# scrose/pylc

Measured on AMD Instinct MI355X. Metric: 512x512 tiles/sec fwd+bwd (DeepLabV3+/ResNet101, 9-class), higher is better.
Workload: dtype f32; 1 GPU; DeepLabV3+ ResNet101 OS16, 3-ch 512x512 tiles, 9 classes, CE+Dice+Focal, clip 0.5 + AdamW, bs=32/GPU (BASELINE.json configs[2]); global_batch=32, parallelism=dp1, conv_arithmetic=f16x3 split (fp32-grade), rccl_ranks=0, wgrad_queue=compute stream, sync_bn=True, activation_format=fp16 planes between BatchNorm and conv kernels (4 B/element)

## Files before the change

### include/pylc_hip.h

```cpp
#ifndef PYLC_HIP_H
#define PYLC_HIP_H

#include <stddef.h>
#include <stdint.h>

#ifdef __cplusplus
extern "C" {
#endif

#define PYLC_OK 0
#define PYLC_ERR_ARG 1
#define PYLC_ERR_HIP 2
#define PYLC_ERR_WORKSPACE 3
#define PYLC_ERR_UNSUPPORTED 4

const char* pylc_last_error(void);
int pylc_abi_version(void);
int pylc_experimental_build(void);
int pylc_init(void);

typedef struct PylcConvDesc {
    int B, H, W;
    int Cin, Cout;
    int R, S;
// ... 280 lines not shown
                            float* losses, void* stream);
int pylc_multiloss_bwd(const float* logits, int pitch, const int64_t* target, long long N, int C,
                       const float* class_weights, const float* stats, double n_global,
                       float w_ce, float w_dice, float w_focal, const float* grad_scale,
                       float* dlogits, int dpitch, unsigned int* amax_bits, void* stream);

size_t pylc_sqnorm_workspace_floats(long long n);
int pylc_grad_norm_clip(const float* g, long long n, float max_norm, float* out2, float* workspace, void* stream);
int pylc_adamw_step(float* p, const float* g, float* m, float* v, long long n, const float* coef,
                    float lr, float beta1, float beta2, float eps, float weight_decay, int step, void* stream);
int pylc_adamw_step_ranges(float* p, const float* g, float* m, float* v, long long n, const float* coef,
                           float lr, float beta1, float beta2, float eps, float weight_decay, int step,
                           const long long* seg_offsets, int seg_count, unsigned int* seg_amax_bits, void* stream);
int pylc_sgd_step(float* p, const float* g, float* buf, long long n, const float* coef, float lr, float momentum,
                  int step, void* stream);

int pylc_dropout(const float* x, int x_pitch, float* out, int out_pitch, long long M, int C, float p,
                 uint64_t seed, void* stream);

#ifdef PYLC_EXPERIMENTAL
int pylc_stream_create_cu_mask(int n_cus, int from_top, void** stream_out);
int pylc_stream_destroy(void* stream);
#endif

int pylc_debug_set_big_tile(int mode);
int pylc_debug_pp_flags(int flags);
int pylc_debug_stagger(int units);
int pylc_debug_dw_tiles(int on);
int pylc_debug_wgrad_m16(int on);
int pylc_debug_wgrad_dma(int on);
int pylc_debug_wgrad_acc1(int on);
int pylc_debug_wgrad_sets(int mode);
int pylc_debug_wgrad_flags(int flags);
int pylc_debug_wgrad_max_steps(int steps);
int pylc_debug_pp_stamps(unsigned long long* buf);

#define PYLC_COMM_ID_BYTES 128
int pylc_comm_available(void);
int pylc_comm_unique_id(void* id_out);
int pylc_comm_init(const void* id, int rank, int world, void** comm_out);
int pylc_comm_allreduce(void* comm, void* buf, long long count, int dtype, void* stream);
int pylc_comm_syncbn_reduce(void* comm, double* moments, int channels, void* stream);
int pylc_comm_destroy(void* comm);

#ifdef __cplusplus
}
#endif
#endif
```

### pylc_amd/csrc/conv_common.h

```cpp
#pragma once
#include "common.h"
#include <type_traits>

namespace pylc {

typedef float f32x4 __attribute__((ext_vector_type(4)));
typedef float f32x16 __attribute__((ext_vector_type(16)));

typedef __bf16 bf16x8 __attribute__((ext_vector_type(8)));

typedef _Float16 f16x8 __attribute__((ext_vector_type(8)));
typedef _Float16 f16x2 __attribute__((ext_vector_type(2)));
typedef float f32x2 __attribute__((ext_vector_type(2)));

constexpr int LDB = 80;

__device__ __forceinline__ void split3(const float (&x)[4], uint2& p0, uint2& p1, uint2& p2) {
    unsigned u0[4], u1[4], u2[4];
#pragma unroll
    for (int e = 0; e < 4; ++e) {
        u0[e] = __float_as_uint(x[e]);
        const float r1 = x[e] - __uint_as_float(u0[e] & 0xFFFF0000u);
        u1[e] = __float_as_uint(r1);
        const float r2 = r1 - __uint_as_float(u1[e] & 0xFFFF0000u);
// ... 106 lines not shown
__device__ __forceinline__ float row_sum16(float v) {
#define PYLC_DPP_ADD(ctrl) v += __builtin_bit_cast(float, __builtin_amdgcn_update_dpp(0, __builtin_bit_cast(int, v), ctrl, 0xF, 0xF, true))
    PYLC_DPP_ADD(0xB1);
    PYLC_DPP_ADD(0x4E);
    PYLC_DPP_ADD(0x141);
    PYLC_DPP_ADD(0x140);
#undef PYLC_DPP_ADD
    return v;
}


struct WgradArgs {
    const float* x;
    const float* dy;
    float* out;
    int M, P, Q;
    int IH, IW, Cin, x_pitch, in_sh, in_sw;
    int TR, TS, dh0, dh_step, dw0, dw_step;
    int N, N_ld, dy_pitch;
    int out_row_stride;
    int tiles_n, tiles_c;
    int splits, m_per_split;
    long long slab_stride;
    const unsigned* amax_dy;
    const unsigned* amax_x;
    long long x_bytes, dy_bytes;
    const void* x_planes;
    const void* dy_planes;
    long long x_plane_stride, dy_plane_stride;
    int nterms;
    int dbg_flags;
};

typedef short s16x4 __attribute__((ext_vector_type(4)));
typedef short s16x8 __attribute__((ext_vector_type(8)));
typedef s16x4 __attribute__((address_space(3))) * lds_s16x4_ptr;

__host__ __device__ constexpr int wg_rowb(int w) { return w * 2 + (w == 32 ? 0 : 64); }

__device__ __forceinline__ bf16x8 tr_frag(const char* p, int rowb) {
    const s16x4 lo = __builtin_amdgcn_ds_read_tr16_b64_v4i16((lds_s16x4_ptr)(p));
    const s16x4 hi = __builtin_amdgcn_ds_read_tr16_b64_v4i16((lds_s16x4_ptr)(p + 4 * rowb));
    const s16x8 v = __builtin_shufflevector(lo, hi, 0, 1, 2, 3, 4, 5, 6, 7);
    return __builtin_bit_cast(bf16x8, v);
}


int launch_wg_pl(WgradArgs& a, int cfg, long long grid, hipStream_t st);
int wgrad_pl_init();

bool takes_pl(const GatherGemmArgs& a);
int launch_gg_pl(GatherGemmArgs& a, hipStream_t st);
int conv_pl_init();
bool takes_stem(const GatherGemmArgs& a);
int launch_stem_fwd(GatherGemmArgs& a, hipStream_t st);
int conv_stem_init();

extern int g_conv_precision;
extern int g_wg_flags;
extern int g_pp_flags;

}
```

### pylc_amd/csrc/conv_igemm.hip

```cpp
#include "conv_common.h"

namespace pylc {

template <int BM, int BN, int WM, int WN, bool CIN4, int PREC>
__global__ __launch_bounds__((BM / WM) * (BN / WN) * 64, 2) void gather_gemm_kernel(const GatherGemmArgs a) {
    constexpr int WAVES_N = BN / WN;
    constexpr int MT = WM / 32, NT = WN / 32;
    constexpr int NTHR = (BM / WM) * (BN / WN) * 64;
    constexpr int RPI = NTHR / 8;
    constexpr int A_IT = BM / RPI, B_IT = BN / RPI;
    static_assert(NTHR == 256 || NTHR == 512, "4 or 8 waves per block");
    static_assert(BM % RPI == 0 && BN % RPI == 0, "tile rows must divide evenly over the loader");
    extern __shared__ __attribute__((aligned(16))) float smem[];
    float* sA = smem;
    float* sB = smem + 2 * BM * LDT;

    const int tile = xcd_remap(blockIdx.x, gridDim.x);
    const int m0 = (tile / a.tiles_n) * BM;
    const int n0 = (tile % a.tiles_n) * BN;
    const int tid = threadIdx.x, lane = tid & 63, wave = tid >> 6;
    const int wave_m = wave / WAVES_N, wave_n = wave % WAVES_N;
    const int v = tid & 7, r0 = tid >> 3;

    int rowh[A_IT], roww[A_IT], rowpix[A_IT];
// ... 1857 lines not shown
        const PylcSlabSum e = tab[lo];
        const long long i = (t - tile_prefix[lo]) * 32 + col;
        f32x4 s = {0.f, 0.f, 0.f, 0.f};
        if (i < e.n4)
            for (int k = sl; k < e.splits; k += 4 * 8) {
                f32x4 v[4];
#pragma unroll
                for (int u = 0; u < 4; ++u) v[u] = *reinterpret_cast<const f32x4*>(e.slabs + (size_t)(k + 8 * u < e.splits ? k + 8 * u : k) * e.slab_stride + 4 * i);
#pragma unroll
                for (int u = 0; u < 4; ++u) { if (k + 8 * u < e.splits) s += v[u]; }
            }
        red[sl][col] = s;
        __syncthreads();
        if (sl == 0 && i < e.n4) {
#pragma unroll
            for (int j = 1; j < 8; ++j) s += red[j][col];
            *reinterpret_cast<f32x4*>(e.dw + 4 * i) = s;
        }
        __syncthreads();
    }
}

extern "C" int pylc_splitk_reduce_batch(const PylcSlabSum* table_dev, const long long* tile_prefix_dev, int n, long long total_tiles, void* stream) {
    PYLC_REQUIRE(table_dev && tile_prefix_dev && n > 0 && total_tiles > 0, "splitk_reduce_batch: bad arguments");
    const int blocks = (int)(total_tiles < 4096 ? total_tiles : 4096);
    hipLaunchKernelGGL(splitk_reduce_batch_kernel, dim3(blocks), dim3(256), 0, as_stream(stream), table_dev, tile_prefix_dev, n, total_tiles);
    PYLC_LAUNCH_CHECK();
    return PYLC_OK;
}

static int wgrad_impl(const PylcConvDesc* d, const float* x, const float* dy, float* dw, float* dbias,
                      void* workspace, size_t workspace_bytes, PylcSlabSum* pending, void* stream);

extern "C" int pylc_conv2d_wgrad(const PylcConvDesc* d, const float* x, const float* dy, float* dw, float* dbias,
                                 void* workspace, size_t workspace_bytes, void* stream) {
    return wgrad_impl(d, x, dy, dw, dbias, workspace, workspace_bytes, nullptr, stream);
}

extern "C" int pylc_conv2d_wgrad_slabs(const PylcConvDesc* d, const float* x, const float* dy, float* dw, void* workspace, size_t workspace_bytes,
                                       PylcSlabSum* pending, void* stream) {
    PYLC_REQUIRE(pending != nullptr, "conv2d_wgrad_slabs: null `pending`");
    return wgrad_impl(d, x, dy, dw, nullptr, workspace, workspace_bytes, pending, stream);
}

static int wgrad_impl(const PylcConvDesc* d, const float* x, const float* dy, float* dw, float* dbias,
                      void* workspace, size_t workspace_bytes, PylcSlabSum* pending, void* stream) {
    if (int rc = check_desc(d)) return rc;
    PYLC_REQUIRE(x && dy && dw, "null pointer");
    PYLC_REQUIRE(dbias == nullptr, "dbias: use pylc_bn_stats on dy (column sums)");
    PYLC_REQUIRE(d->x_fmt == d->dy_fmt, "conv2d_wgrad: x and dy must be in the same format (both fp32 or both fp16 planes; pylc_to_planes converts)");
    hipStream_t st = as_stream(stream);
    const WgradPlan p = plan_wgrad(d);
    const size_t need = p.splits > 1 ? (size_t)p.splits * p.slab * sizeof(float) : 0;
    if (need > workspace_bytes || (need && !workspace))
        return fail(PYLC_ERR_WORKSPACE, "wgrad workspace too small: need %zu bytes, got %zu", need, workspace_bytes);
    PYLC_REQUIRE(p.slab % 4 == 0, "dw size must be a multiple of 4");
    const int T = d->R * d->S;
    WgradArgs a{};
    a.x = x; a.dy = dy; a.out = p.splits > 1 ? static_cast<float*>(workspace) : dw;
    a.P = d->OH; a.Q = d->OW; a.M = d->B * d->OH * d->OW;
    a.IH = d->H; a.IW = d->W; a.Cin = d->Cin; a.x_pitch = d->x_pitch; a.in_sh = a.in_sw = d->stride;
    a.TR = d->R; a.TS = d->S; a.dh0 = -d->pad; a.dh_step = d->dil; a.dw0 = -d->pad; a.dw_step = d->dil;
    a.N = d->Cout; a.N_ld = roundup4(d->Cout); a.dy_pitch = d->y_pitch;
    PYLC_REQUIRE(a.N_ld <= d->y_pitch, "dy pitch must cover roundup4(Cout)");
    a.out_row_stride = T * d->Cin;
    a.tiles_n = p.tiles_n; a.tiles_c = p.tiles_c; a.splits = p.splits; a.m_per_split = p.m_per_split;
    a.slab_stride = p.slab;
    PYLC_REQUIRE(g_conv_precision < 2 || (d->dy_amax && d->x_amax), "f16x3 / fp16 mode: conv2d_wgrad needs dy_amax and x_amax in the descriptor");
    a.x_bytes = (((long long)d->B * d->H * d->W - 1) * d->x_pitch + d->Cin) * 4;
    a.dy_bytes = (((long long)d->B * d->OH * d->OW - 1) * d->y_pitch + a.N_ld) * 4;
    a.amax_dy = d->dy_amax; a.amax_x = d->x_amax;
    const long long grid = (long long)p.tiles_n * p.tiles_c * (p.cin4 ? 1 : T) * p.splits;
    int rc;
    if (d->x_fmt == 1) {
        PYLC_REQUIRE(g_conv_precision >= 2 && !p.cin4 && d->Cout % 8 == 0, "conv2d_wgrad: fp16-plane operands need precision mode 2 or 3, "
                     "a dense geometry and Cout %% 8 == 0");
        a.x_planes = x; a.dy_planes = dy; a.x = nullptr; a.dy = nullptr;
        a.x_plane_stride = planes_stride_rule((long long)d->B * d->H * d->W, d->Cin, d->x_pitch, (g_conv_precision == 3 ? 1 : 2));
        a.dy_plane_stride = planes_stride_rule((long long)d->B * d->OH * d->OW, d->Cout, d->y_pitch, (g_conv_precision == 3 ? 1 : 2));
        a.N_ld = d->Cout;
        a.x_bytes /= 2; a.dy_bytes = (((long long)d->B * d->OH * d->OW - 1) * d->y_pitch + a.N_ld) * 2;
        a.nterms = g_conv_precision == 3 ? 1 : 3;
        rc = launch_wg_pl(a, p.cfg, grid, st);
    } else
    switch (p.cfg) {
        case 0: rc = launch_wg<128, 128, 64, 64, false>(a, grid, st); break;
        case 1: rc = launch_wg<64, 64, 32, 32, false>(a, grid, st); break;
        case 2: rc = launch_wg<32, 128, 32, 32, false>(a, grid, st); break;
        default: rc = launch_wg<64, 64, 32, 32, true>(a, grid, st); break;
    }
    if (rc) return rc;
    if (pending != nullptr) {
        *pending = PylcSlabSum{p.splits > 1 ? static_cast<const float*>(workspace) : nullptr, dw, p.slab / 4, p.slab, p.splits > 1 ? p.splits : 0, 0};
        return PYLC_OK;
    }
    if (p.splits > 1) {
        const long long n4 = p.slab / 4;
        const int blocks = (int)(cdiv<long long>(n4, 32) < 4096 ? cdiv<long long>(n4, 32) : 4096);
        hipLaunchKernelGGL(splitk_reduce_kernel, dim3(blocks), dim3(256), 0, st, static_cast<const float*>(workspace), dw, n4,
                           p.splits, p.slab);
// ... 14 lines not shown
```

### pylc_amd/csrc/wgrad_pl.hip

```cpp
#include "conv_common.h"

namespace pylc {

typedef __attribute__((address_space(3))) void* wg_lds_vptr;
template <int BN, int BC, int WN, int WC, int NTERMS, int FAST, bool ACC1 = false, int SETS = 1, bool M16 = false, bool DMA = false>
__global__ __launch_bounds__(256, ACC1 ? 4 : 2) void wgrad_pl_kernel(const WgradArgs a) {
    static_assert(!DMA || (M16 && SETS == 1), "DMA: the 16x16x32 image only");
    constexpr int NPL = NTERMS == 3 ? 2 : 1;
    constexpr int WAVES_C = BC / WC;
    constexpr int NT = WN / 32, CT = WC / 32;
    static_assert(!M16 || (BN == 128 && BC == 128 && WN == 64 && WC == 64 && !ACC1), "M16: 128 x 128 block tiles, 64 x 64 wave tiles, two accumulator sets");
    constexpr int VA = BN / 8, RA = 256 / VA, IA = 32 / RA > 0 ? 32 / RA : 1;
    constexpr int VB = BC / 8, RB = 256 / VB, IB = 32 / RB > 0 ? 32 / RB : 1;
    constexpr bool A_ALL = RA <= 32, B_ALL = RB <= 32;
    constexpr int ROWA = M16 ? 256 : wg_rowb(BN), ROWB = M16 ? 256 : wg_rowb(BC);
    constexpr int PLA = 32 * ROWA, PLB = 32 * ROWB;
    static_assert((BN / WN) * (BC / WC) == 4, "4 waves per block");
    static_assert(FAST == 1 || FAST == 2, "buffer-load geometry paths only");
    extern __shared__ __attribute__((aligned(16))) float smem[];
    char* sA = reinterpret_cast<char*>(smem);
    char* sB = sA + NPL * PLA;
    constexpr int STG = NPL * (PLA + PLB);

    const int T = a.TR * a.TS;
    int id = (a.dbg_flags & 1) ? (int)blockIdx.x : xcd_remap(blockIdx.x, gridDim.x);
    int tc, tn, tap, split;
    if (a.dbg_flags & 2) {
        split = id % a.splits; id /= a.splits;
        tc = id % a.tiles_c; id /= a.tiles_c;
        tn = id % a.tiles_n; id /= a.tiles_n;
        tap = id;
    } else if (a.dbg_flags & 4) {
        tc = id % a.tiles_c; id /= a.tiles_c;
        tn = id % a.tiles_n; id /= a.tiles_n;
        tap = id % T; id /= T;
        split = id;
    } else if (a.Cin > a.N && !(a.dbg_flags & 8)) {
        tap = id % T; id /= T;
        tn = id % a.tiles_n; id /= a.tiles_n;
        tc = id % a.tiles_c; id /= a.tiles_c;
        split = id;
    } else {
        tap = id % T; id /= T;
        tc = id % a.tiles_c; id /= a.tiles_c;
        tn = id % a.tiles_n; id /= a.tiles_n;
        split = id;
    }
    const int n0 = tn * BN, c0 = tc * BC;
    const int m_begin = split * a.m_per_split;
    const int m_end = min(a.M, m_begin + a.m_per_split);
    const int S = (m_end - m_begin + 31) / 32;

    const int tid = threadIdx.x, lane = tid & 63, wave = tid >> 6;
    const int wave_n = wave / WAVES_C, wave_c = wave % WAVES_C;
    const int va = tid % VA, pra = tid / VA;
    const int vb = tid % VB, prb = tid / VB;
    const int sw_row = ((pra & 3) << 2) | ((pra >> 2) & 3);
    const int va_g = DMA ? (va ^ sw_row) : va, vb_g = DMA ? (vb ^ sw_row) : vb;
    const int dh = a.dh0 + (tap / a.TS) * a.dh_step, dw = a.dw0 + (tap % a.TS) * a.dw_step;
    const bool b_col_ok = c0 + 8 * vb_g < a.Cin && (B_ALL || prb < 32);
    const bool a_col_ok = n0 + 8 * va_g < a.N_ld && (A_ALL || pra < 32);

    f32x16 acc[M16 ? 1 : NT][M16 ? 1 : CT];
    constexpr bool TWO_ACC = NTERMS == 3 && !ACC1;
    f32x16 acc_lo[TWO_ACC && !M16 ? NT : 1][TWO_ACC && !M16 ? CT : 1];
    f32x4 acc16[M16 ? 4 : 1][M16 ? 4 : 1], acc16_lo[M16 && TWO_ACC ? 4 : 1][M16 && TWO_ACC ? 4 : 1];
    if constexpr (M16) {
#pragma unroll
        for (int i = 0; i < 4; ++i)
#pragma unroll
            for (int j = 0; j < 4; ++j) {
                acc16[i][j] = f32x4{0.f, 0.f, 0.f, 0.f};
                if constexpr (TWO_ACC) acc16_lo[i][j] = f32x4{0.f, 0.f, 0.f, 0.f};
            }
    } else {
#pragma unroll
    for (int i = 0; i < NT; ++i)
#pragma unroll
        for (int j = 0; j < CT; ++j)
#pragma unroll
            for (int r = 0; r < 16; ++r) {
                acc[i][j][r] = 0.f;
                if constexpr (TWO_ACC) acc_lo[i][j][r] = 0.f;
            }
    }
    const float scale_a = pow2_scale_for(*a.amax_dy), scale_b = pow2_scale_for(*a.amax_x);

    constexpr unsigned OOB = 0xFFFFFFF0u;
    const bool il_dy = NPL == 2 && planes_il(a.dy_plane_stride), il_x = NPL == 2 && planes_il(a.x_plane_stride);
    const unsigned mdy = (unsigned)__builtin_amdgcn_readfirstlane(il_dy ? 2 : 1), mx = (unsigned)__builtin_amdgcn_readfirstlane(il_x ? 2 : 1);
    auto colh = [](unsigned c, bool il) { return il ? ((c >> 5) << 6) + (c & 31u) : c; };
    const __amdgpu_buffer_rsrc_t rdy0 = __builtin_amdgcn_make_buffer_rsrc(const_cast<void*>(a.dy_planes), 0, (int)((unsigned)a.dy_bytes * mdy), 0x00020000);
    const __amdgpu_buffer_rsrc_t rdy1 = __builtin_amdgcn_make_buffer_rsrc(
        const_cast<char*>(static_cast<const char*>(a.dy_planes) + a.dy_plane_stride * 2), 0, (int)((unsigned)a.dy_bytes * mdy - (il_dy ? 64u : 0u)), 0x00020000);
    const __amdgpu_buffer_rsrc_t rx0 = __builtin_amdgcn_make_buffer_rsrc(const_cast<void*>(a.x_planes), 0, (int)((unsigned)a.x_bytes * mx), 0x00020000);
    const __amdgpu_buffer_rsrc_t rx1 = __builtin_amdgcn_make_buffer_rsrc(
        const_cast<char*>(static_cast<const char*>(a.x_planes) + a.x_plane_stride * 2), 0, (int)((unsigned)a.x_bytes * mx - (il_x ? 64u : 0u)), 0x00020000);

    constexpr int NSET = SETS;
    uint4 ra[NSET][IA][NPL], rb[NSET][IB][NPL];
    int f_mb = m_begin, f_q0 = 0, f_p = 0, f_b = 0;
    unsigned f_va[IA], f_tx[IB];
    int f_wc[IB];
    int g_q[FAST == 2 ? IB : 1], g_p[FAST == 2 ? IB : 1], g_b[FAST == 2 ? IB : 1];
    if constexpr (FAST == 2) {
#pragma unroll
        for (int i = 0; i < IB; ++i) {
            const int m = m_begin + prb + RB * i;
            g_q[i] = m % a.Q;
            const int t = m / a.Q;
            g_p[i] = t % a.P;
            g_b[i] = t / a.P;
        }
    }
    {
        f_q0 = m_begin % a.Q;
        const int t = m_begin / a.Q;
        f_p = t % a.P;
        f_b = t / a.P;
#pragma unroll
        for (int i = 0; i < IA; ++i) f_va[i] = a_col_ok ? ((unsigned)(pra + RA * i) * (unsigned)a.dy_pitch * mdy + colh((unsigned)(n0 + 8 * va_g), il_dy)) * 2u : OOB;
#pragma unroll
        for (int i = 0; i < IB; ++i) {
            f_tx[i] = ((unsigned)((prb + RB * i) * a.in_sw) * (unsigned)a.x_pitch * mx + colh((unsigned)(c0 + 8 * vb_g), il_x)) * 2u;
            f_wc[i] = (prb + RB * i) * a.in_sw + dw;
        }
    }
    char* dma_a = nullptr; char* dma_b = nullptr;
    if constexpr (DMA) { dma_a = sA + (4 * wave) * 256; dma_b = sB + (4 * wave) * 256; }
    auto ldp = [&](const __amdgpu_buffer_rsrc_t& r0, const __amdgpu_buffer_rsrc_t& r1, unsigned voff, unsigned soff, uint4 (&dst)[NPL], char* lds0, int plb) {
        if constexpr (DMA) {
            __builtin_amdgcn_raw_ptr_buffer_load_lds(r0, (wg_lds_vptr)lds0, 16, voff, soff, 0, 0);
            if constexpr (NPL == 2) __builtin_amdgcn_raw_ptr_buffer_load_lds(r1, (wg_lds_vptr)(lds0 + plb), 16, voff, soff, 0, 0);
        } else {
            dst[0] = __builtin_bit_cast(uint4, __builtin_amdgcn_raw_buffer_load_b128(r0, voff, soff, 0));
            if constexpr (NPL == 2) dst[1] = __builtin_bit_cast(uint4, __builtin_amdgcn_raw_buffer_load_b128(r1, voff, soff, 0));
        }
    };
    auto load_tile = [&](auto setc) {
        constexpr int set = DMA ? 0 : decltype(setc)::value;
        constexpr int stg = DMA ? decltype(setc)::value * STG : 0;
        const unsigned soff = (unsigned)__builtin_amdgcn_readfirstlane((int)((unsigned)f_mb * (unsigned)a.dy_pitch * 2u * mdy));
        if constexpr (FAST == 2) {
            const unsigned colb = colh((unsigned)(c0 + 8 * vb_g), il_x);
#pragma unroll
            for (int i = 0; i < IB; ++i) {
                const int hi = g_p[i] * a.in_sh + dh, wi = g_q[i] * a.in_sw + dw;
                const bool ok = b_col_ok & (f_mb + prb + RB * i < m_end) & ((unsigned)hi < (unsigned)a.IH) & ((unsigned)wi < (unsigned)a.IW);
                const unsigned off = (((unsigned)(g_b[i] * a.IH + hi) * (unsigned)a.IW + (unsigned)wi) * (unsigned)a.x_pitch * mx + colb) * 2u;
                ldp(rx0, rx1, ok ? off : OOB, 0u, rb[set][i], dma_b + stg + RB * i * 256, PLB);
                g_q[i] += 32;
                while (g_q[i] >= a.Q) { g_q[i] -= a.Q; ++g_p[i]; }
                while (g_p[i] >= a.P) { g_p[i] -= a.P; ++g_b[i]; }
            }
#pragma unroll
            for (int i = 0; i < IA; ++i) {
                const bool ok = f_mb + pra + RA * i < m_end;
                ldp(rdy0, rdy1, ok ? f_va[i] : OOB, soff, ra[set][i], dma_a + stg + RA * i * 256, PLA);
            }
            f_mb += 32;
            return;
        }
        const int hi = f_p * a.in_sh + dh;
        const bool row_ok = b_col_ok && (unsigned)hi < (unsigned)a.IH;
        const unsigned delta = (unsigned)((((f_b * a.IH + hi) * a.IW + f_q0 * a.in_sw + dw) * a.x_pitch) * 2) * mx;
        const int wq = f_q0 * a.in_sw;
#pragma unroll
        for (int i = 0; i < IB; ++i) {
            const bool ok = row_ok & ((unsigned)(f_wc[i] + wq) < (unsigned)a.IW);
            ldp(rx0, rx1, ok ? f_tx[i] + delta : OOB, 0u, rb[set][i], dma_b + stg + RB * i * 256, PLB);
        }
#pragma unroll
        for (int i = 0; i < IA; ++i) ldp(rdy0, rdy1, f_va[i], soff, ra[set][i], dma_a + stg + RA * i * 256, PLA);
        f_mb += 32;
        f_q0 += 32;
        if (f_q0 == a.Q) {
            f_q0 = 0;
            if (++f_p == a.P) { f_p = 0; ++f_b; }
        }
    };
    auto store_tile = [&](auto setc) {
        constexpr int set = decltype(setc)::value;
        if constexpr (M16) {
            const int sa = ((pra & 3) << 2) | ((pra >> 2) & 3);
#pragma unroll
            for (int i = 0; i < IA; ++i)
#pragma unroll
                for (int pl = 0; pl < NPL; ++pl) *reinterpret_cast<uint4*>(sA + pl * PLA + (pra + RA * i) * 256 + 16 * (va ^ sa)) = ra[set][i][pl];
#pragma unroll
            for (int i = 0; i < IB; ++i)
#pragma unroll
                for (int pl = 0; pl < NPL; ++pl) *reinterpret_cast<uint4*>(sB + pl * PLB + (prb + RB * i) * 256 + 16 * (vb ^ sa)) = rb[set][i][pl];
            return;
        }
        if (A_ALL || pra < 32) {
#pragma unroll
            for (int i = 0; i < IA; ++i)
#pragma unroll
                for (int pl = 0; pl < NPL; ++pl) *reinterpret_cast<uint4*>(sA + pl * PLA + (pra + RA * i) * ROWA + 16 * va) = ra[set][i][pl];
        }
        if (B_ALL || prb < 32) {
#pragma unroll
            for (int i = 0; i < IB; ++i)
#pragma unroll
                for (int pl = 0; pl < NPL; ++pl) *reinterpret_cast<uint4*>(sB + pl * PLB + (prb + RB * i) * ROWB + 16 * vb) = rb[set][i][pl];
        }
    };
    const int g = lane >> 4, h = g >> 1, q4 = (lane & 15) >> 2, p4 = lane & 3;
    const char* fa_base = sA + (8 * h + q4) * ROWA + 2 * (wave_n * WN + 16 * (g & 1) + 4 * p4);
    const char* fb_base = sB + (8 * h + q4) * ROWB + 2 * (wave_c * WC + 16 * (g & 1) + 4 * p4);

    const int swz_lo = (q4 << 2) | ((2 * g) & 3);
    const int m16_a0 = (8 * g + q4) * 256 + 16 * ((wave_n * 8 + (p4 >> 1)) ^ swz_lo) + 8 * (p4 & 1);
    const int m16_b0 = (8 * g + q4) * 256 + 16 * ((wave_c * 8 + (p4 >> 1)) ^ swz_lo) + 8 * (p4 & 1);
    auto tr16 = [&](const char* base, int off0, int t) {
        const int o = off0 ^ (32 * t);
        const s16x4 lo = __builtin_amdgcn_ds_read_tr16_b64_v4i16((lds_s16x4_ptr)(base + o));
        const s16x4 hi = __builtin_amdgcn_ds_read_tr16_b64_v4i16((lds_s16x4_ptr)(base + ((o + 1024) ^ 16)));
        return __builtin_bit_cast(f16x8, __builtin_shufflevector(lo, hi, 0, 1, 2, 3, 4, 5, 6, 7));
    };
    auto compute_tile16 = [&](auto stgc) {
        constexpr int so = decltype(stgc)::value * STG;
        f16x8 fa[4][NPL];
#pragma unroll
        for (int t = 0; t < 4; ++t)
#pragma unroll
            for (int pl = 0; pl < NPL; ++pl) fa[t][pl] = tr16(sA + so + pl * PLA, m16_a0, t);
#pragma unroll
        for (int j = 0; j < 4; ++j) {
            f16x8 fb[NPL];
#pragma unroll
            for (int pl = 0; pl < NPL; ++pl) fb[pl] = tr16(sB + so + pl * PLB, m16_b0, j);
            if constexpr (NTERMS == 3) {
#pragma unroll
                for (int i = 0; i < 4; ++i) acc16_lo[i][j] = __builtin_amdgcn_mfma_f32_16x16x32_f16(fa[i][NPL - 1], fb[0], acc16_lo[i][j], 0, 0, 0);
#pragma unroll
                for (int i = 0; i < 4; ++i) acc16_lo[i][j] = __builtin_amdgcn_mfma_f32_16x16x32_f16(fa[i][0], fb[NPL - 1], acc16_lo[i][j], 0, 0, 0);
            }
#pragma unroll
            for (int i = 0; i < 4; ++i) acc16[i][j] = __builtin_amdgcn_mfma_f32_16x16x32_f16(fa[i][0], fb[0], acc16[i][j], 0, 0, 0);
        }
    };
    [[maybe_unused]] auto step_dma = [&](auto stgc, auto issue) {
        constexpr int so = decltype(stgc)::value * STG;
        f16x8 fa[4][NPL], fb[4][NPL];
#pragma unroll
        for (int t = 0; t < 4; ++t)
#pragma unroll
            for (int pl = 0; pl < NPL; ++pl) {
                fa[t][pl] = tr16(sA + so + pl * PLA, m16_a0, t);
                fb[t][pl] = tr16(sB + so + pl * PLB, m16_b0, t);
            }
        __builtin_amdgcn_sched_barrier(0);
        issue();
        __builtin_amdgcn_sched_barrier(0);
#pragma unroll
        for (int j = 0; j < 4; ++j) {
            if constexpr (NTERMS == 3) {
#pragma unroll
                for (int i = 0; i < 4; ++i) acc16_lo[i][j] = __builtin_amdgcn_mfma_f32_16x16x32_f16(fa[i][NPL - 1], fb[j][0], acc16_lo[i][j], 0, 0, 0);
#pragma unroll
                for (int i = 0; i < 4; ++i) acc16_lo[i][j] = __builtin_amdgcn_mfma_f32_16x16x32_f16(fa[i][0], fb[j][NPL - 1], acc16_lo[i][j], 0, 0, 0);
            }
#pragma unroll
            for (int i = 0; i < 4; ++i) acc16[i][j] = __builtin_amdgcn_mfma_f32_16x16x32_f16(fa[i][0], fb[j][0], acc16[i][j], 0, 0, 0);
        }
    };
    unsigned ad_a[4][2], ad_b[4][2];
    {
        const unsigned la0 = (unsigned)(uintptr_t)(wg_lds_vptr)sA, lb0 = (unsigned)(uintptr_t)(wg_lds_vptr)sB;
#pragma unroll
        for (int t = 0; t < 4; ++t) {
            ad_a[t][0] = la0 + (unsigned)(m16_a0 ^ (32 * t)); ad_a[t][1] = la0 + (unsigned)((m16_a0 ^ (32 * t)) ^ 16);
            ad_b[t][0] = lb0 + (unsigned)(m16_b0 ^ (32 * t)); ad_b[t][1] = lb0 + (unsigned)((m16_b0 ^ (32 * t)) ^ 16);
        }
    }
    auto tr16_asm = [&](const unsigned (&ad)[2], auto offc) {
        constexpr int off = decltype(offc)::value;
        unsigned long long lo, hi;
        asm volatile("ds_read_b64_tr_b16 %0, %1 offset:%2" : "=v"(lo) : "v"(ad[0]), "n"(off) : "memory");
        asm volatile("ds_read_b64_tr_b16 %0, %1 offset:%2" : "=v"(hi) : "v"(ad[1]), "n"(off + 1024) : "memory");
        return ulonglong2{lo, hi};
    };
    auto step_dma_early = [&](auto stgc, auto issue) {
        constexpr int so = decltype(stgc)::value * STG;
        __builtin_amdgcn_sched_barrier(0);
        issue();
        __builtin_amdgcn_sched_barrier(0);
        ulonglong2 ua[4][NPL], ub[4][NPL];
        auto rd = [&](auto tc, auto plc) {
            constexpr int t = decltype(tc)::value, pl = decltype(plc)::value;
            ua[t][pl] = tr16_asm(ad_a[t], std::integral_constant<int, so + pl * PLA>{});
            ub[t][pl] = tr16_asm(ad_b[t], std::integral_constant<int, so + pl * PLB>{});
        };
        typedef std::integral_constant<int, 0> I0; typedef std::integral_constant<int, 1> I1;
        typedef std::integral_constant<int, 2> I2; typedef std::integral_constant<int, 3> I3;
        rd(I0{}, I0{}); if constexpr (NPL == 2) rd(I0{}, I1{});
        rd(I1{}, I0{}); if constexpr (NPL == 2) rd(I1{}, I1{});
        rd(I2{}, I0{}); if constexpr (NPL == 2) rd(I2{}, I1{});
        rd(I3{}, I0{}); if constexpr (NPL == 2) rd(I3{}, I1{});
        asm volatile("s_waitcnt lgkmcnt(0)" ::: "memory");
#pragma unroll
        for (int t = 0; t < 4; ++t)
#pragma unroll
            for (int pl = 0; pl < NPL; ++pl) asm volatile("" : "+v"(ua[t][pl].x), "+v"(ua[t][pl].y), "+v"(ub[t][pl].x), "+v"(ub[t][pl].y));
        __builtin_amdgcn_sched_barrier(0);
        f16x8 fa[4][NPL], fb[4][NPL];
#pragma unroll
        for (int t = 0; t < 4; ++t)
#pragma unroll
            for (int pl = 0; pl < NPL; ++pl) { fa[t][pl] = __builtin_bit_cast(f16x8, ua[t][pl]); fb[t][pl] = __builtin_bit_cast(f16x8, ub[t][pl]); }
#pragma unroll
        for (int j = 0; j < 4; ++j) {
            if constexpr (NTERMS == 3) {
#pragma unroll
                for (int i = 0; i < 4; ++i) acc16_lo[i][j] = __builtin_amdgcn_mfma_f32_16x16x32_f16(fa[i][NPL - 1], fb[j][0], acc16_lo[i][j], 0, 0, 0);
#pragma unroll
                for (int i = 0; i < 4; ++i) acc16_lo[i][j] = __builtin_amdgcn_mfma_f32_16x16x32_f16(fa[i][0], fb[j][NPL - 1], acc16_lo[i][j], 0, 0, 0);
            }
#pragma unroll
            for (int i = 0; i < 4; ++i) acc16[i][j] = __builtin_amdgcn_mfma_f32_16x16x32_f16(fa[i][0], fb[j][0], acc16[i][j], 0, 0, 0);
        }
    };
    auto compute_tile = [&]() {
        if constexpr (M16) { compute_tile16(std::integral_constant<int, 0>{}); return; }
#pragma unroll
        for (int ks = 0; ks < 2; ++ks) {
            bf16x8 fa[NT][NPL], fb[CT][NPL];
#pragma unroll
            for (int i = 0; i < NT; ++i)
#pragma unroll
                for (int pl = 0; pl < NPL; ++pl) fa[i][pl] = tr_frag(fa_base + pl * PLA + 16 * ks * ROWA + 64 * i, ROWA);
#pragma unroll
            for (int j = 0; j < CT; ++j)
#pragma unroll
                for (int pl = 0; pl < NPL; ++pl) fb[j][pl] = tr_frag(fb_base + pl * PLB + 16 * ks * ROWB + 64 * j, ROWB);
            if constexpr (NTERMS == 3 && ACC1) {
                const _Float16 k11 = (_Float16)(1.f / 2048.f);
                f16x8 a1s[NT], b1s[CT];
#pragma unroll
                for (int i = 0; i < NT; ++i) a1s[i] = __builtin_bit_cast(f16x8, fa[i][1]) * k11;
#pragma unroll
                for (int j = 0; j < CT; ++j) b1s[j] = __builtin_bit_cast(f16x8, fb[j][1]) * k11;
#pragma unroll
                for (int i = 0; i < NT; ++i)
#pragma unroll
// ... 40 lines not shown
            load_tile(Set0{});
            for (int s = 0; s < S; s += 2) {
                __syncthreads();
                step_dma_early(Set0{}, [&] { if (s + 1 < S) load_tile(Stg1{}); });
                if (s + 1 < S) {
                    __syncthreads();
                    step_dma_early(Stg1{}, [&] { if (s + 2 < S) load_tile(Set0{}); });
                }
            }
        }
    } else
    if (S > 0) {
        int s = 0;
        load_tile(Set0{});
        if constexpr (NSET == 2) {
            load_tile(Set1{});
            for (; s + 1 < S; s += 2) {
                step(Set0{}, s);
                step(Set1{}, s + 1);
            }
            if (s < S) step(Set0{}, s);
        } else {
            for (; s < S; ++s) step(Set0{}, s);
        }
    }

    const float unscale_a = 1.f / scale_a, unscale_b = 1.f / scale_b;
    float* out = a.out + (size_t)split * a.slab_stride;
    const int col_base = tap * a.Cin;
    if constexpr (M16) {
        const float us = unscale_a * unscale_b;
#pragma unroll
        for (int j = 0; j < 4; ++j) {
            const int c = c0 + wave_c * WC + j * 16 + (lane & 15);
            if (c >= a.Cin) continue;
#pragma unroll
            for (int i = 0; i < 4; ++i)
#pragma unroll
                for (int r = 0; r < 4; ++r) {
                    const int n = n0 + wave_n * WN + i * 16 + 4 * (lane >> 4) + r;
                    float val = acc16[i][j][r];
                    if constexpr (TWO_ACC) val = (val + acc16_lo[i][j][r] * (1.f / 2048.f)) * unscale_a * unscale_b;
                    else val = val * unscale_a * unscale_b;
                    (void)us;
                    if (n < a.N) out[(size_t)n * a.out_row_stride + col_base + c] = val;
                }
        }
        return;
    }
#pragma unroll
    for (int j = 0; j < CT; ++j) {
        const int c = c0 + wave_c * WC + j * 32 + (lane & 31);
        if (c >= a.Cin) continue;
#pragma unroll
        for (int i = 0; i < NT; ++i) {
#pragma unroll
            for (int r = 0; r < 16; ++r) {
                const int n = n0 + wave_n * WN + i * 32 + (r & 3) + 8 * (r >> 2) + 4 * (lane >> 5);
                float val = acc[i][j][r];
                if constexpr (TWO_ACC) val = (val + acc_lo[i][j][r] * (1.f / 2048.f)) * unscale_a * unscale_b;
                else val = val * unscale_a * unscale_b;
                if (n < a.N) out[(size_t)n * a.out_row_stride + col_base + c] = val;
            }
        }
    }
}

template <int BN, int BC, int NTERMS>
// ... 33 lines not shown
            return PYLC_OK;
        }
        if (a.nterms == 3 && (g_wg_m16 == 2 || (g_wg_m16 == 1 && a.TR * a.TS == 1))) {
            constexpr size_t lds = 4 * 32 * 256;
            if (g_wg_dma) {
                if (fast == 1) hipLaunchKernelGGL((wgrad_pl_kernel<BN, BC, WN, WC, 3, 1, false, 1, true, true>), g, b, 2 * lds, st, a);
                else hipLaunchKernelGGL((wgrad_pl_kernel<BN, BC, WN, WC, 3, 2, false, 1, true, true>), g, b, 2 * lds, st, a);
                PYLC_LAUNCH_CHECK();
                return PYLC_OK;
            }
            if (fast == 1) hipLaunchKernelGGL((wgrad_pl_kernel<BN, BC, WN, WC, 3, 1, false, 1, true>), g, b, lds, st, a);
            else hipLaunchKernelGGL((wgrad_pl_kernel<BN, BC, WN, WC, 3, 2, false, 1, true>), g, b, lds, st, a);
            PYLC_LAUNCH_CHECK();
            return PYLC_OK;
        }
    }
    if (a.nterms == 1) {
        constexpr size_t lds = wgpl_smem<BN, BC, 1>();
        if (two) {
            if (fast == 1) hipLaunchKernelGGL((wgrad_pl_kernel<BN, BC, WN, WC, 1, 1, false, 2>), g, b, lds, st, a);
            else hipLaunchKernelGGL((wgrad_pl_kernel<BN, BC, WN, WC, 1, 2, false, 2>), g, b, lds, st, a);
        } else if (fast == 1) hipLaunchKernelGGL((wgrad_pl_kernel<BN, BC, WN, WC, 1, 1>), g, b, lds, st, a);
        else hipLaunchKernelGGL((wgrad_pl_kernel<BN, BC, WN, WC, 1, 2>), g, b, lds, st, a);
    } else {
        constexpr size_t lds = wgpl_smem<BN, BC, 3>();
        if (two) {
            if (fast == 1) hipLaunchKernelGGL((wgrad_pl_kernel<BN, BC, WN, WC, 3, 1, false, 2>), g, b, lds, st, a);
            else hipLaunchKernelGGL((wgrad_pl_kernel<BN, BC, WN, WC, 3, 2, false, 2>), g, b, lds, st, a);
        } else if (fast == 1) hipLaunchKernelGGL((wgrad_pl_kernel<BN, BC, WN, WC, 3, 1>), g, b, lds, st, a);
        else hipLaunchKernelGGL((wgrad_pl_kernel<BN, BC, WN, WC, 3, 2>), g, b, lds, st, a);
    }
    PYLC_LAUNCH_CHECK();
    return PYLC_OK;
}

int launch_wg_pl(WgradArgs& a, int cfg, long long grid, hipStream_t st) {
    a.dbg_flags = g_wg_flags;
    PYLC_REQUIRE(grid > 0 && grid < (1ll << 31), "wgrad grid out of range");
    PYLC_REQUIRE(a.x_planes && a.dy_planes && a.amax_dy && a.amax_x, "wgrad (fp16-plane operands): null planes / ranges");
    PYLC_REQUIRE(a.Q >= 16 && a.Cin % 8 == 0 && a.N_ld % 8 == 0 && a.x_pitch % 8 == 0 && a.dy_pitch % 8 == 0,
                 "wgrad (fp16-plane operands): needs OW >= 16 and channel counts / pitches that are multiples of 8");
    PYLC_REQUIRE(a.x_bytes < 0xFFFFFFF0ll && a.dy_bytes < 0xFFFFFFF0ll, "wgrad (fp16-plane operands): a plane must stay below 4 GiB");
    switch (cfg) {
        case 0: return launch_cfg<128, 128, 64, 64>(a, grid, st);
        case 1: return launch_cfg<64, 64, 32, 32>(a, grid, st);
        default: return launch_cfg<32, 128, 32, 32>(a, grid, st);
    }
}

template <typename K>
static hipError_t opt_in(K kernel, size_t bytes) {
    return hipFuncSetAttribute(reinterpret_cast<const void*>(kernel), hipFuncAttributeMaxDynamicSharedMemorySize, (int)bytes);
}

int wgrad_pl_init() {
#define PYLC_OPT(BN, BC, WN, WC)                                                                      \
    PYLC_HIP(opt_in(wgrad_pl_kernel<BN, BC, WN, WC, 3, 1>, wgpl_smem<BN, BC, 3>()));                  \
    PYLC_HIP(opt_in(wgrad_pl_kernel<BN, BC, WN, WC, 3, 2>, wgpl_smem<BN, BC, 3>()));                  \
    PYLC_HIP(opt_in(wgrad_pl_kernel<BN, BC, WN, WC, 1, 1>, wgpl_smem<BN, BC, 1>()));                  \
    PYLC_HIP(opt_in(wgrad_pl_kernel<BN, BC, WN, WC, 1, 2>, wgpl_smem<BN, BC, 1>()));                  \
    PYLC_HIP(opt_in((wgrad_pl_kernel<BN, BC, WN, WC, 3, 1, false, 2>), wgpl_smem<BN, BC, 3>()));      \
    PYLC_HIP(opt_in((wgrad_pl_kernel<BN, BC, WN, WC, 3, 2, false, 2>), wgpl_smem<BN, BC, 3>()));      \
    PYLC_HIP(opt_in((wgrad_pl_kernel<BN, BC, WN, WC, 1, 1, false, 2>), wgpl_smem<BN, BC, 1>()));      \
    PYLC_HIP(opt_in((wgrad_pl_kernel<BN, BC, WN, WC, 1, 2, false, 2>), wgpl_smem<BN, BC, 1>()));
    PYLC_OPT(128, 128, 64, 64)
    PYLC_HIP(opt_in((wgrad_pl_kernel<128, 128, 64, 64, 3, 1, false, 1, true, true>), 2 * 4 * 32 * 256));
// ... 11 lines not shown
```

### pylc_amd/lib.py

```python
import ctypes as C
import os

import torch

_HERE = os.path.dirname(os.path.abspath(__file__))
LIB_PATH = os.environ.get('PYLC_LIB') or os.path.join(_HERE, 'libpylc_hip.so')

ABI_VERSION = 15


class PylcError(RuntimeError):
    pass


class ConvDesc(C.Structure):
    _fields_ = [(n, C.c_int) for n in ('B', 'H', 'W', 'Cin', 'Cout', 'R', 'S', 'stride', 'pad', 'dil',
                                       'OH', 'OW', 'x_pitch', 'y_pitch')] + \
               [(n, C.c_void_p) for n in ('x_amax', 'w_amax', 'dy_amax',
                                          'w_planes', 'w_planes_t')] + \
               [(n, C.c_int) for n in ('x_fmt', 'dy_fmt', 'out_fmt')] + [('out_bound', C.c_void_p)] + \
               [('w_planes_fmt', C.c_int)]


class WPrepEntry(C.Structure):
# ... 18 lines not shown


class FwdEp(C.Structure):
    _fields_ = [('scale', C.c_void_p), ('shift', C.c_void_p), ('scale_amax', C.c_void_p), ('shift_amax', C.c_void_p), ('residual', C.c_void_p),
                ('res_fmt', C.c_int), ('res_scale_bound', C.c_void_p), ('res_amax', C.c_void_p), ('x_true_amax', C.c_void_p), ('relu', C.c_int),
                ('amax_out', C.c_void_p)]


class DwDesc(C.Structure):
    _fields_ = [(n, C.c_int) for n in ('B', 'H', 'W', 'C', 'stride', 'dil', 'OH', 'OW', 'x_pitch', 'y_pitch')]


_P = C.c_void_p
_I = C.c_int
_LL = C.c_longlong
_F = C.c_float
_D = C.c_double
_SZ = C.c_size_t

SIGNATURES = {
    'pylc_last_error': (C.c_char_p, []),
    'pylc_abi_version': (_I, []),
    'pylc_planes_stride': (_LL, [_LL, _I, _I]),
    'pylc_set_planes_interleave': (_I, [_I]),
    'pylc_experimental_build': (_I, []),
    'pylc_init': (_I, []),
    'pylc_set_conv_precision': (_I, [_I]),
    'pylc_get_conv_precision': (_I, []),
    'pylc_debug_set_big_tile': (_I, [_I]),
    'pylc_debug_pp_flags': (_I, [_I]),
    'pylc_debug_stagger': (_I, [_I]),
    'pylc_debug_wgrad_flags': (_I, [_I]),
    'pylc_debug_wgrad_max_steps': (_I, [_I]),
    'pylc_comm_available': (_I, []),
    'pylc_comm_unique_id': (_I, [_P]),
    'pylc_comm_init': (_I, [_P, _I, _I, C.POINTER(C.c_void_p)]),
    'pylc_comm_allreduce': (_I, [_P, _P, _LL, _I, _P]),
    'pylc_comm_syncbn_reduce': (_I, [_P, _P, _I, _P]),
    'pylc_comm_destroy': (_I, [_P]),
    'pylc_debug_dw_tiles': (_I, [_I]),
    'pylc_range_product': (_I, [_P, _P, _F, _P, _P, _P]),
    'pylc_maxpool_fwd_planes': (_I, [_P, _P, _LL, _I, _P, _P, _I, _I, _I, _I, _I, _I, _I, _I, _I, _P]),
    'pylc_upsample2_crop_concat_planes': (_I, [_P, _I, _I, _I, _I, _I, _P, _I, _I, _I, _I, _P, _LL, _I, _P, _P]),
    'pylc_conv1x1_fold_input_affine': (_I, [_P, _P, _P, _P, _I, _I, _P, _P, _P, _P]),
    'pylc_debug_wgrad_acc1': (_I, [_I]),
    'pylc_debug_wgrad_sets': (_I, [_I]),
    'pylc_debug_wgrad_m16': (_I, [_I]),
    'pylc_debug_wgrad_dma': (_I, [_I]),
    'pylc_debug_pp_stamps': (_I, [_P]),
    'pylc_amax': (_I, [_P, _LL, _I, _I, _P, _P]),
    'pylc_amax_segments': (_I, [_P, _P, _I, _P, _P]),
    'pylc_to_planes': (_I, [_P, _I, _P, _I, _LL, _LL, _I, _P, _I, _P]),
    'pylc_from_planes': (_I, [_P, _I, _LL, _P, _I, _LL, _I, _P, _I, _P]),
    'pylc_planes_colsum_workspace_floats': (C.c_size_t, [_I]),
    'pylc_planes_colsum': (_I, [_P, _I, _LL, _I, _P, _LL, _I, _P, _P, _P]),
    'pylc_weight_prepare': (_I, [_P, _P, _I, _LL, _P, _P, _I, _P]),
    'pylc_conv2d_dgrad_needs_f32_weights': (_I, [C.POINTER(ConvDesc)]),
    'pylc_conv2d_fwd': (_I, [C.POINTER(ConvDesc), _P, _P, _P, _P, _P]),
    'pylc_conv2d_fwd_bnact': (_I, [C.POINTER(ConvDesc), _P, _P, _P, _P, _P, _P, _I, _P, _P, _P]),
    'pylc_conv2d_fwd_bnact_ex': (_I, [C.POINTER(ConvDesc), _P, _P, _P, C.POINTER(FwdEp), _P, _P]),
    'pylc_conv2d_fwd_stats_floats': (_SZ, [C.POINTER(ConvDesc)]),
    'pylc_conv2d_fwd_stats': (_I, [C.POINTER(ConvDesc), _P, _P, _P, _P, _P, C.POINTER(_I), _P]),
    'pylc_conv2d_dgrad': (_I, [C.POINTER(ConvDesc), _P, _P, _P, _I, _P]),
    'pylc_conv2d_dgrad_add': (_I, [C.POINTER(ConvDesc), _P, _P, _P, _I, _P, _P, _P]),
    'pylc_relu_bwd_bits': (_I, [_P, _P, _P, _LL, _I, _P]),
    'pylc_conv2d_dgrad_bn_floats': (_SZ, [C.POINTER(ConvDesc)]),
# ... 157 lines not shown
```

Baseline: 435.1 tiles/s.

## Skip padding-only rows and out-of-range channel groups in wgrad plane kernel

For the FAST==1 wgrad path, computes per-tap the range of output rows whose input row lands inside the image and iterates K-steps only over those live rows, jumping over dead rows in the fetch cursor. In the M16 path it splits the channel tile among waves by the channels actually present, skipping MFMA work and LDS reads for groups beyond Cin. It also raises launch-bounds occupancy for the single-term DMA variant and adds a debug query that counts live versus total K-steps. This removes wasted MFMA and load work on zero-padded borders, mainly for dilated 3x3 convs in ASPP. The cost is extra per-block setup arithmetic and more complex cursor logic that must stay consistent across splits.

```diff
diff --git a/include/pylc_hip.h b/include/pylc_hip.h
--- a/include/pylc_hip.h
+++ b/include/pylc_hip.h
@@ -336,6 +336,7 @@
 int pylc_debug_wgrad_acc1(int on);
 int pylc_debug_wgrad_sets(int mode);
 int pylc_debug_wgrad_flags(int flags);
+int pylc_debug_wgrad_ksteps(const PylcConvDesc* d, long long* live, long long* total);
 int pylc_debug_wgrad_max_steps(int steps);
 int pylc_debug_pp_stamps(unsigned long long* buf);
 
diff --git a/pylc_amd/csrc/conv_common.h b/pylc_amd/csrc/conv_common.h
--- a/pylc_amd/csrc/conv_common.h
+++ b/pylc_amd/csrc/conv_common.h
@@ -162,6 +162,23 @@
     int dbg_flags;
 };
 
+__host__ __device__ inline void wg_live_rows(const WgradArgs& a, int dh, int& p0, int& np) {
+    p0 = 0; np = a.P;
+    if (a.dbg_flags & 16) return;
+    if (dh < 0) p0 = (-dh + a.in_sh - 1) / a.in_sh;
+    int p1 = a.IH - 1 - dh < 0 ? -1 : (a.IH - 1 - dh) / a.in_sh;
+    if (p1 > a.P - 1) p1 = a.P - 1;
+    np = p1 >= p0 ? p1 - p0 + 1 : 0;
+    if (np == 0) p0 = 0;
+}
+__host__ __device__ inline int wg_live_before(int t, int tq, int P, int p0, int np) {
+    const int r = t / tq, part = t - r * tq;
+    const int b = r / P, p = r - b * P;
+    const int in = p - p0;
+    const int rows = b * np + (in < 0 ? 0 : in > np ? np : in);
+    return rows * tq + (in >= 0 && in < np ? part : 0);
+}
+
 typedef short s16x4 __attribute__((ext_vector_type(4)));
 typedef short s16x8 __attribute__((ext_vector_type(8)));
 typedef s16x4 __attribute__((address_space(3))) * lds_s16x4_ptr;
@@ -178,6 +195,7 @@
 
 int launch_wg_pl(WgradArgs& a, int cfg, long long grid, hipStream_t st);
 int wgrad_pl_init();
+void wg_pl_ksteps(WgradArgs& a, long long* live, long long* total);
 
 bool takes_pl(const GatherGemmArgs& a);
 int launch_gg_pl(GatherGemmArgs& a, hipStream_t st);
diff --git a/pylc_amd/csrc/conv_igemm.hip b/pylc_amd/csrc/conv_igemm.hip
--- a/pylc_amd/csrc/conv_igemm.hip
+++ b/pylc_amd/csrc/conv_igemm.hip
@@ -1913,6 +1913,29 @@
 static int wgrad_impl(const PylcConvDesc* d, const float* x, const float* dy, float* dw, float* dbias,
                       void* workspace, size_t workspace_bytes, PylcSlabSum* pending, void* stream);
 
+static void wgrad_geometry(const PylcConvDesc* d, const WgradPlan& p, WgradArgs& a) {
+    a.P = d->OH; a.Q = d->OW; a.M = d->B * d->OH * d->OW;
+    a.IH = d->H; a.IW = d->W; a.Cin = d->Cin; a.x_pitch = d->x_pitch; a.in_sh = a.in_sw = d->stride;
+    a.TR = d->R; a.TS = d->S; a.dh0 = -d->pad; a.dh_step = d->dil; a.dw0 = -d->pad; a.dw_step = d->dil;
+    a.N = d->Cout; a.N_ld = roundup4(d->Cout); a.dy_pitch = d->y_pitch;
+    a.out_row_stride = d->R * d->S * d->Cin;
+    a.tiles_n = p.tiles_n; a.tiles_c = p.tiles_c; a.splits = p.splits; a.m_per_split = p.m_per_split;
+    a.slab_stride = p.slab;
+}
+
+extern "C" int pylc_debug_wgrad_ksteps(const PylcConvDesc* d, long long* live, long long* total) {
+    if (int rc = check_desc(d)) return rc;
+    PYLC_REQUIRE(live && total, "wgrad_ksteps: null result pointer");
+    const WgradPlan p = plan_wgrad(d);
+    WgradArgs a{};
+    wgrad_geometry(d, p, a);
+    if (d->x_fmt == 1 && !p.cin4 && d->OW >= 16) { wg_pl_ksteps(a, live, total); return PYLC_OK; }
+    long long tot = 0;
+    for (int s = 0; s < p.splits; ++s) tot += (std::min(a.M, (s + 1) * p.m_per_split) - s * p.m_per_split + 31) / 32;
+    *live = *total = tot * p.tiles_n * p.tiles_c * (p.cin4 ? 1 : d->R * d->S);
+    return PYLC_OK;
+}
+
 extern "C" int pylc_conv2d_wgrad(const PylcConvDesc* d, const float* x, const float* dy, float* dw, float* dbias,
                                  void* workspace, size_t workspace_bytes, void* stream) {
     return wgrad_impl(d, x, dy, dw, dbias, workspace, workspace_bytes, nullptr, stream);
@@ -1939,14 +1962,8 @@
     const int T = d->R * d->S;
     WgradArgs a{};
     a.x = x; a.dy = dy; a.out = p.splits > 1 ? static_cast<float*>(workspace) : dw;
-    a.P = d->OH; a.Q = d->OW; a.M = d->B * d->OH * d->OW;
-    a.IH = d->H; a.IW = d->W; a.Cin = d->Cin; a.x_pitch = d->x_pitch; a.in_sh = a.in_sw = d->stride;
-    a.TR = d->R; a.TS = d->S; a.dh0 = -d->pad; a.dh_step = d->dil; a.dw0 = -d->pad; a.dw_step = d->dil;
-    a.N = d->Cout; a.N_ld = roundup4(d->Cout); a.dy_pitch = d->y_pitch;
+    wgrad_geometry(d, p, a);
     PYLC_REQUIRE(a.N_ld <= d->y_pitch, "dy pitch must cover roundup4(Cout)");
-    a.out_row_stride = T * d->Cin;
-    a.tiles_n = p.tiles_n; a.tiles_c = p.tiles_c; a.splits = p.splits; a.m_per_split = p.m_per_split;
-    a.slab_stride = p.slab;
     PYLC_REQUIRE(g_conv_precision < 2 || (d->dy_amax && d->x_amax), "f16x3 / fp16 mode: conv2d_wgrad needs dy_amax and x_amax in the descriptor");
     a.x_bytes = (((long long)d->B * d->H * d->W - 1) * d->x_pitch + d->Cin) * 4;
     a.dy_bytes = (((long long)d->B * d->OH * d->OW - 1) * d->y_pitch + a.N_ld) * 4;
diff --git a/pylc_amd/csrc/wgrad_pl.hip b/pylc_amd/csrc/wgrad_pl.hip
--- a/pylc_amd/csrc/wgrad_pl.hip
+++ b/pylc_amd/csrc/wgrad_pl.hip
@@ -4,7 +4,7 @@
 
 typedef __attribute__((address_space(3))) void* wg_lds_vptr;
 template <int BN, int BC, int WN, int WC, int NTERMS, int FAST, bool ACC1 = false, int SETS = 1, bool M16 = false, bool DMA = false>
-__global__ __launch_bounds__(256, ACC1 ? 4 : 2) void wgrad_pl_kernel(const WgradArgs a) {
+__global__ __launch_bounds__(256, (ACC1 || (NTERMS == 1 && FAST == 1 && DMA)) ? 4 : 2) void wgrad_pl_kernel(const WgradArgs a) {
     static_assert(!DMA || (M16 && SETS == 1), "DMA: the 16x16x32 image only");
     constexpr int NPL = NTERMS == 3 ? 2 : 1;
     constexpr int WAVES_C = BC / WC;
@@ -49,15 +49,23 @@
     const int n0 = tn * BN, c0 = tc * BC;
     const int m_begin = split * a.m_per_split;
     const int m_end = min(a.M, m_begin + a.m_per_split);
-    const int S = (m_end - m_begin + 31) / 32;
-
     const int tid = threadIdx.x, lane = tid & 63, wave = tid >> 6;
     const int wave_n = wave / WAVES_C, wave_c = wave % WAVES_C;
+    const int dh = a.dh0 + (tap / a.TS) * a.dh_step, dw = a.dw0 + (tap % a.TS) * a.dw_step;
+    int S = (m_end - m_begin + 31) / 32;
+    int live_p0 = 0, live_np = a.P;
+    if constexpr (FAST == 1) {
+        wg_live_rows(a, dh, live_p0, live_np);
+        const int tq = a.Q >> 5;
+        S = __builtin_amdgcn_readfirstlane(wg_live_before(m_end >> 5, tq, a.P, live_p0, live_np) - wg_live_before(m_begin >> 5, tq, a.P, live_p0, live_np));
+        live_p0 = __builtin_amdgcn_readfirstlane(live_p0);
+        live_np = __builtin_amdgcn_readfirstlane(live_np);
+    }
+    const int live_p1 = live_p0 + live_np, dead_px = (a.P - live_np) * a.Q;
     const int va = tid % VA, pra = tid / VA;
     const int vb = tid % VB, prb = tid / VB;
     const int sw_row = ((pra & 3) << 2) | ((pra >> 2) & 3);
     const int va_g = DMA ? (va ^ sw_row) : va, vb_g = DMA ? (vb ^ sw_row) : vb;
-    const int dh = a.dh0 + (tap / a.TS) * a.dh_step, dw = a.dw0 + (tap % a.TS) * a.dw_step;
     const bool b_col_ok = c0 + 8 * vb_g < a.Cin && (B_ALL || prb < 32);
     const bool a_col_ok = n0 + 8 * va_g < a.N_ld && (A_ALL || pra < 32);
 
@@ -118,6 +126,11 @@
         const int t = m_begin / a.Q;
         f_p = t % a.P;
         f_b = t / a.P;
+        if constexpr (FAST == 1) {
+            if (f_p < live_p0) { f_p = live_p0; f_q0 = 0; }
+            else if (f_p >= live_p1) { f_p = live_p0; f_q0 = 0; ++f_b; }
+            f_mb = (f_b * a.P + f_p) * a.Q + f_q0;
+        }
 #pragma unroll
         for (int i = 0; i < IA; ++i) f_va[i] = a_col_ok ? ((unsigned)(pra + RA * i) * (unsigned)a.dy_pitch * mdy + colh((unsigned)(n0 + 8 * va_g), il_dy)) * 2u : OOB;
 #pragma unroll
@@ -176,7 +189,7 @@
         f_q0 += 32;
         if (f_q0 == a.Q) {
             f_q0 = 0;
-            if (++f_p == a.P) { f_p = 0; ++f_b; }
+            if (++f_p == live_p1) { f_p = live_p0; ++f_b; f_mb += dead_px; }
         }
     };
     auto store_tile = [&](auto setc) {
@@ -212,9 +225,16 @@
 
     const int swz_lo = (q4 << 2) | ((2 * g) & 3);
     const int m16_a0 = (8 * g + q4) * 256 + 16 * ((wave_n * 8 + (p4 >> 1)) ^ swz_lo) + 8 * (p4 & 1);
-    const int m16_b0 = (8 * g + q4) * 256 + 16 * ((wave_c * 8 + (p4 >> 1)) ^ swz_lo) + 8 * (p4 & 1);
-    auto tr16 = [&](const char* base, int off0, int t) {
-        const int o = off0 ^ (32 * t);
+    int m16_gb = 4 * wave_c, m16_ng = 4;
+    if constexpr (M16) {
+        if (!(a.dbg_flags & 16)) {
+            const int L = min(8, (a.Cin - c0 + 15) >> 4), h0 = (L + 1) >> 1;
+            m16_gb = __builtin_amdgcn_readfirstlane(wave_c * h0);
+            m16_ng = __builtin_amdgcn_readfirstlane(wave_c ? L - h0 : h0);
+        }
+    }
+    auto m16_boff = [&](int t) { return (8 * g + q4) * 256 + 16 * ((2 * (m16_gb + t) + (p4 >> 1)) ^ swz_lo) + 8 * (p4 & 1); };
+    auto tr16 = [&](const char* base, int o) {
         const s16x4 lo = __builtin_amdgcn_ds_read_tr16_b64_v4i16((lds_s16x4_ptr)(base + o));
         const s16x4 hi = __builtin_amdgcn_ds_read_tr16_b64_v4i16((lds_s16x4_ptr)(base + ((o + 1024) ^ 16)));
         return __builtin_bit_cast(f16x8, __builtin_shufflevector(lo, hi, 0, 1, 2, 3, 4, 5, 6, 7));
@@ -225,12 +245,13 @@
 #pragma unroll
         for (int t = 0; t < 4; ++t)
 #pragma unroll
-            for (int pl = 0; pl < NPL; ++pl) fa[t][pl] = tr16(sA + so + pl * PLA, m16_a0, t);
+            for (int pl = 0; pl < NPL; ++pl) fa[t][pl] = tr16(sA + so + pl * PLA, m16_a0 ^ (32 * t));
 #pragma unroll
         for (int j = 0; j < 4; ++j) {
+            if (j >= m16_ng) break;
             f16x8 fb[NPL];
 #pragma unroll
-            for (int pl = 0; pl < NPL; ++pl) fb[pl] = tr16(sB + so + pl * PLB, m16_b0, j);
+            for (int pl = 0; pl < NPL; ++pl) fb[pl] = tr16(sB + so + pl * PLB, m16_boff(j));
             if constexpr (NTERMS == 3) {
 #pragma unroll
                 for (int i = 0; i < 4; ++i) acc16_lo[i][j] = __builtin_amdgcn_mfma_f32_16x16x32_f16(fa[i][NPL - 1], fb[0], acc16_lo[i][j], 0, 0, 0);
@@ -248,14 +269,15 @@
         for (int t = 0; t < 4; ++t)
 #pragma unroll
             for (int pl = 0; pl < NPL; ++pl) {
-                fa[t][pl] = tr16(sA + so + pl * PLA, m16_a0, t);
-                fb[t][pl] = tr16(sB + so + pl * PLB, m16_b0, t);
+                fa[t][pl] = tr16(sA + so + pl * PLA, m16_a0 ^ (32 * t));
+                fb[t][pl] = tr16(sB + so + pl * PLB, m16_boff(t));
             }
         __builtin_amdgcn_sched_barrier(0);
         issue();
         __builtin_amdgcn_sched_barrier(0);
 #pragma unroll
         for (int j = 0; j < 4; ++j) {
+            if (j >= m16_ng) break;
             if constexpr (NTERMS == 3) {
 #pragma unroll
                 for (int i = 0; i < 4; ++i) acc16_lo[i][j] = __builtin_amdgcn_mfma_f32_16x16x32_f16(fa[i][NPL - 1], fb[j][0], acc16_lo[i][j], 0, 0, 0);
@@ -272,7 +294,7 @@
 #pragma unroll
         for (int t = 0; t < 4; ++t) {
             ad_a[t][0] = la0 + (unsigned)(m16_a0 ^ (32 * t)); ad_a[t][1] = la0 + (unsigned)((m16_a0 ^ (32 * t)) ^ 16);
-            ad_b[t][0] = lb0 + (unsigned)(m16_b0 ^ (32 * t)); ad_b[t][1] = lb0 + (unsigned)((m16_b0 ^ (32 * t)) ^ 16);
+            ad_b[t][0] = lb0 + (unsigned)m16_boff(t); ad_b[t][1] = lb0 + (unsigned)(m16_boff(t) ^ 16);
         }
     }
     auto tr16_asm = [&](const unsigned (&ad)[2], auto offc) {
@@ -312,6 +334,7 @@
             for (int pl = 0; pl < NPL; ++pl) { fa[t][pl] = __builtin_bit_cast(f16x8, ua[t][pl]); fb[t][pl] = __builtin_bit_cast(f16x8, ub[t][pl]); }
 #pragma unroll
         for (int j = 0; j < 4; ++j) {
+            if (j >= m16_ng) break;
             if constexpr (NTERMS == 3) {
 #pragma unroll
                 for (int i = 0; i < 4; ++i) acc16_lo[i][j] = __builtin_amdgcn_mfma_f32_16x16x32_f16(fa[i][NPL - 1], fb[j][0], acc16_lo[i][j], 0, 0, 0);
@@ -418,8 +441,8 @@
         const float us = unscale_a * unscale_b;
 #pragma unroll
         for (int j = 0; j < 4; ++j) {
-            const int c = c0 + wave_c * WC + j * 16 + (lane & 15);
-            if (c >= a.Cin) continue;
+            const int c = c0 + (m16_gb + j) * 16 + (lane & 15);
+            if (j >= m16_ng || c >= a.Cin) continue;
 #pragma unroll
             for (int i = 0; i < 4; ++i)
 #pragma unroll
@@ -519,6 +542,25 @@
     }
     PYLC_LAUNCH_CHECK();
     return PYLC_OK;
+}
+
+void wg_pl_ksteps(WgradArgs& a, long long* live, long long* total) {
+    a.dbg_flags = g_wg_flags;
+    const bool fast1 = a.Q % 32 == 0;
+    long long lv = 0, tot = 0;
+    for (int split = 0; split < a.splits; ++split) {
+        const int m_begin = split * a.m_per_split, m_end = a.M < m_begin + a.m_per_split ? a.M : m_begin + a.m_per_split;
+        const int steps = (m_end - m_begin + 31) / 32;
+        for (int tap = 0; tap < a.TR * a.TS; ++tap) {
+            tot += steps;
+            if (!fast1) { lv += steps; continue; }
+            int p0, np;
+            wg_live_rows(a, a.dh0 + (tap / a.TS) * a.dh_step, p0, np);
+            lv += wg_live_before(m_end >> 5, a.Q >> 5, a.P, p0, np) - wg_live_before(m_begin >> 5, a.Q >> 5, a.P, p0, np);
+        }
+    }
+    *live = lv * a.tiles_n * a.tiles_c;
+    *total = tot * a.tiles_n * a.tiles_c;
 }
 
 int launch_wg_pl(WgradArgs& a, int cfg, long long grid, hipStream_t st) {
diff --git a/pylc_amd/lib.py b/pylc_amd/lib.py
--- a/pylc_amd/lib.py
+++ b/pylc_amd/lib.py
@@ -74,6 +74,7 @@
     'pylc_debug_stagger': (_I, [_I]),
     'pylc_debug_wgrad_flags': (_I, [_I]),
     'pylc_debug_wgrad_max_steps': (_I, [_I]),
+    'pylc_debug_wgrad_ksteps': (_I, [C.POINTER(ConvDesc), C.POINTER(_LL), C.POINTER(_LL)]),
     'pylc_comm_available': (_I, []),
     'pylc_comm_unique_id': (_I, [_P]),
     'pylc_comm_init': (_I, [_P, _I, _I, C.POINTER(C.c_void_p)]),
```

Result: no change. 437.5 tiles/s (median of 6 runs) (+0.6%).
